# fahmyadan/SMARTS

Hardware: AMD Instinct MI355X
Metric: aggregate env-steps/s (all agents) (higher is better)
Workload: dtype f64; 1 GPU; scenarios/loop, 4096 batched envs x 32 Laner agents, waypoints(4x20, lookahead 32)+neighbours(10, r=50 m) obs, OGM 64x64 @ 50/64 m/px, dt=0.1, auto-reset (BASELINE.json configs[3]); total_envs=4096, envs_per_gpu=4096, vehicles_per_env=32, launch_form=large_one_lane

## Files before the change

### smarts_amd/csrc/smx_kernels.hip

```cpp
#include <hip/hip_runtime.h>

#include <algorithm>
#include <cmath>
#include <cstdio>
#include <cstdlib>
#include <cstring>
#include <new>
#include <string>
#include <vector>

#include "smx_guard.h"
#include "smx_history.h"
#include "smx_host.h"
#include "smx_plan.h"
#include "smx_scan.h"
#include "smx_vehicle.h"

#define SMX_COLLISION_LEEWAY 0.05
#define SMX_POSE_SCAN_RADIUS 10.0
#define SMX_WPT_PRELOAD 8
#define SMX_SLOW_BLOCKS 512

struct KernelArgs {
  smx_config cfg;
  MapDev map;
  smx_state st;
  smx_spawns sp;
  smx_outputs out;
  const int8_t* actions;
  const float* actions_f32;
  const double* traj;
  const int32_t* traj_n;
  int traj_max;
  const uint8_t* env_mask;
  const double* lidar_rays;
  const smx_via* vias;
  const int32_t* via_slot_off;
  int first_only;
  int keep_reward_done;
  int reset_all;
  double heading_gain_pos, lateral_gain_pos;
  int wp_pool_limit;
  char* wp_spill;
  int walk_new;
  double nb_d2_max;
  int debug_skip;
  int wp_blocks, obs_blocks, lidar_blocks;
  double dagm_reach;
  uint8_t* rgb;
  KnotLists knots;
  const KnotRow* knot_table;
  unsigned long long* knot_served;
  MissionsDev missions;
  const int32_t* alive_list;
  const int32_t* alive_count;
  int alive_segmented;
  int32_t* status;
  double* seeds_carry;
  double* facts_carry;
  int32_t* slow_list;
  int32_t* slow_count;
  uint8_t* seed_pending;
  uint8_t* guard;
  GuardBox guard_box;
  HistoryDev history;
  HistoryDimsDev dims;
};
enum {
  SMX_DEVICE_BAD_LANE_ACTION = 1,
  SMX_DEVICE_BAD_TRAJECTORY = 2,
  SMX_DEVICE_BAD_TARGET_POSE = 4
};

#define SF(field) a.st.f64[(size_t)(field) * total + gid]

#define SMX_SEG_STRIDE 32
__device__ __forceinline__ size_t seg_position(const size_t seg, const size_t off) {
  return ((off >> 6) << 9) | (seg << 6) | (off & 63);
}

__device__ __forceinline__ size_t launch_vehicle(const KernelArgs& a, size_t i, size_t total) {
  if (a.alive_list == nullptr) return i < total ? i : total;
  const int32_t entry = a.alive_list[i < total ? i : total - 1];
  if (a.alive_segmented) {
// ... 1060 lines not shown
              const double d = first_waypoint_distance(rx[q], ry[q], rdx[q], rdy[q], kn_n[q], px, py);
              if (d < my_d) {
                my_d = d;
                my_idx = __popc(started);
              }
              started |= 1 << q;
            }
          }
          const int n_paths = __popc(started);
          if (!slow && n_paths > 0) {
            const int want = wanted_path(my_idx, la.lane_change, n_paths);
#pragma unroll
            for (int q = 0; q < SMX_WP_LANES; ++q)
              if ((started >> q) & 1)
                if (__popc(started & ((1 << q) - 1)) == want) qw = q;
            int n32w = 0, nk16 = 0, last = -1, stw = 0;
            smx_lp_rec r0 = smx_lp_rec{};
#pragma unroll
            for (int q = 0; q < SMX_WP_LANES; ++q)
              if (q == qw) {
                stw = st[q];
                n32w = kn_n[q];
                nk16 = kn_nk16[q];
                last = kn_end16[q];
                r0.x = rx[q];
                r0.y = ry[q];
                r0.dirx = rdx[q];
                r0.diry = rdy[q];
                r0.heading = rh[q];
              }
            r0.lane = 0;
            const int n16 = n32w < SMX_CTRL_WPS ? n32w : SMX_CTRL_WPS;
            double* col = path_lds + threadIdx.x;
            const int32_t* const knot1 = table ? a.knot_table[stw].idx : a.knots.idx + paths + gid * SMX_WP_LANES + qw;
            ctrl_waypoints_from_knots<true>(a, knot1, table ? (size_t)1 : paths, r0, nk16, last, n16, px, py,
                                            [&](int i, const WaypointOut& w) {
                                              col[(size_t)i * SMX_BLOCK] = w.heading;
                                              if (i < CTRL_XY) {
                                                col[(size_t)(SMX_CTRL_WPS + i) * SMX_BLOCK] = w.x;
                                                col[(size_t)(SMX_CTRL_WPS + CTRL_XY + i) * SMX_BLOCK] = w.y;
                                              }
                                            });
            path.n = n16;
#pragma unroll
            for (int k = 0; k < SMX_CTRL_WPS; ++k) {
              const bool held = k < n16;
              path.h[k] = held ? col[(size_t)k * SMX_BLOCK] : 0.0;
              path.x[k] = (held && k < CTRL_XY) ? col[(size_t)(SMX_CTRL_WPS + (k < CTRL_XY ? k : 0)) * SMX_BLOCK] : 0.0;
              path.y[k] = (held && k < CTRL_XY) ? col[(size_t)(SMX_CTRL_WPS + CTRL_XY + (k < CTRL_XY ? k : 0)) * SMX_BLOCK] : 0.0;
            }
          }
        }
      }
      if (!slow) {
        ControlOut co = idle_command(cs);
        if (has_action) {
          if (path.n > 0 && !SMX_SKIP(a, 1 << 28)) {
            co = lane_following_from_path(s, cs, c.dt, la.target_speed, la.lane_change, la.hg, la.lg, path);
          } else {
            co = last_command(cs);
          }
        }
        SF(SMX_S_PREV_X) = s.x;
        SF(SMX_S_PREV_Y) = s.y;
        if (!SMX_SKIP(a, 1 << 27)) vehicle_step(s, co, c.dt);
        if (!GUARD || guard_before_store(a, gid, flags, s)) store_vehicle_state(a, gid, total, s, cs, flags);
      }
    }
  }
  const unsigned long long mask = __ballot(slow);
  if (mask != 0ull) {
    const int lane = threadIdx.x & 63;
    int base = 0;
    if (lane == __ffsll((long long)mask) - 1) base = atomicAdd(a.slow_count, __popcll(mask));
    base = __shfl(base, __ffsll((long long)mask) - 1);
// ... 756 lines not shown
  const size_t path = gid * SMX_WP_LANES + p0;
  const int flags = a.st.flags[gid];
  int n = 0, nk = 0, cnt = 0;
  double D = 0.0;
  if (honour_pending && a.seed_pending != nullptr && a.seed_pending[gid]) return;
  if ((flags & SMX_F_ALIVE) && !(flags & SMX_F_SOCIAL) && (!a.first_only || whatever_the_pass || (flags & SMX_F_FIRST))) {
    const PathSeeds seed = load_seeds(a, gid, total);
    if (seed.road >= 0 && seed.n_lanes <= SMX_WP_LANES && p0 < seed.n_lanes) {
      const double px = SF(SMX_S_X), py = SF(SMX_S_Y);
      const int start = seed_start(m, seed, p0, px, py);
      if (start >= 0) {
        a.knots.idx[path] = start;
        const KnotListHead w = walk_knot_list(m, seed.f, start, c.wp_lookahead, SMX_CTRL_WPS, px, py,
                                              [&](int k, int idx, double) { a.knots.idx[(size_t)k * paths + path] = idx; });
        n = w.n;
        nk = w.nk;
        D = w.D;
        cnt = w.cnt;
        a.knots.nk16[path] = (uint8_t)w.nk16;
        a.knots.end16[path] = w.end16;
        a.knots.key[path] = start;
        a.knots.key[paths + path] = seed.f.n > 0 ? seed.f.road[0] : -1;
        a.knots.key[2 * paths + path] = seed.f.n > 1 ? seed.f.road[1] : -1;
      }
    }
  }
  a.knots.n[path] = (int16_t)n;
  a.knots.nk[path] = (int16_t)nk;
  a.knots.cnt[path] = (uint8_t)cnt;
  a.knots.D[path] = D;
  if (n == 0) a.knots.key[path] = -1;
}

__global__ void __launch_bounds__(SMX_BLOCK) k_knot_table(const MapDev m, const int lookahead, KnotRow* rows, int32_t* stats) {
  const int lp = (int)(blockIdx.x * SMX_BLOCK + threadIdx.x);
  if (lp >= m.n_lanepoints) return;
  KnotRow row;
  build_knot_row(m, lp, lookahead, SMX_CTRL_WPS, row);
  rows[lp] = row;
  if (row.flags & SMX_KROW_TABLED) atomicAdd(stats, 1);
  if (row.flags & SMX_KROW_SINGLE_ROAD) atomicAdd(stats + 1, 1);
}

__global__ void __launch_bounds__(SMX_BLOCK) k_wp_walk(const KernelArgs a) {
  SMX_TSTAMP(span0);
  const size_t total = (size_t)a.cfg.num_envs * a.cfg.num_vehicles;
  const size_t lane_no = (size_t)blockIdx.x * SMX_BLOCK + threadIdx.x;
  wp_walk_for(a, launch_vehicle(a, lane_no / SMX_WP_LANES, total), (int)(lane_no % SMX_WP_LANES), true);
  SMX_TSTAMP(span1);
  SMX_TSPAN(3, span0, span1);
}

__global__ void __launch_bounds__(SMX_BLOCK) k_wp_walk_listed(const KernelArgs a) {
  const int count = *a.slow_count;
  constexpr int VPB = SMX_BLOCK / SMX_WP_LANES;
  for (int i = (int)blockIdx.x * VPB + (int)threadIdx.x / SMX_WP_LANES; i < count; i += (int)gridDim.x * VPB)
    wp_walk_for(a, (size_t)a.slow_list[i], (int)threadIdx.x % SMX_WP_LANES, false);
}

struct __align__(16) WpStageCell {
  float heading, width, speed;
  short lane;
  signed char lane_index;
  signed char pad;
};

__device__ __forceinline__ void waypoints_tables_role(const KernelArgs& a, const int block) {
  extern __shared__ __align__(16) unsigned char stage_raw[];
  __shared__ WpRowBook book;
  const smx_config& c = a.cfg;
  const MapDev& m = a.map;
  const smx_outputs& o = a.out;
// ... 156 lines not shown
      } else {
        n_paths_total = wp_emit_branches<SMX_BLOCK>(a, seed.f, gid, p0, px, py, knots, cnt > 0 ? a.knots.idx[path] : -1, cnt, -1, g);
        fw = team_first_waypoint(tm.started, g, n_paths_total > 0);
      }
      wp_close_rows(a, gid, p0, n_paths_total);
    } else {
      if (tm.staged && !tm.listed) {
        BranchState bs;
        bs.reset();
        wp_emit_path<SMX_BLOCK>(a, seed.f, bs, a.knots.idx[path], gid, px, py, knots, tm.my_row ? tm.prov : 0, tm.my_row, true, &g, false);
      }
      fw = team_first_waypoint(tm.started, g, tm.n_paths > 0);
    }
  }
  SMX_TSTAMP(tw5);
  SMX_TACC(5, tw4, tw5);
  if (live && p0 == 0) trip_meter_update<SMX_BLOCK>(a, gid, total, flags, px, py, knots, fw);
  SMX_TSTAMP(tw6);
  SMX_TACC(3, tw0, tw6);
}

#define SMX_WPE_KNOTS 10
#ifndef SMX_WPE_POOL
#define SMX_WPE_POOL 352
#endif
struct __align__(8) WpKnot {
  double x, y, h, cum;
};
struct WpKnotLanes {
  short lane, strict;
};
#define SMX_WPE_SPILL_GROUP_BYTES ((size_t)SMX_BLOCK * (SMX_WPE_KNOTS + 1) * (sizeof(WpKnot) + sizeof(WpKnotLanes)))

__device__ __forceinline__ void waypoints_emit_role(const KernelArgs& a, const int block) {
  __shared__ WpKnot pool[SMX_WPE_POOL];
  __shared__ WpKnotLanes pool_lanes[SMX_WPE_POOL];
  __shared__ WpRowBook book;
  __shared__ double hdr_step[SMX_BLOCK], hdr_D[SMX_BLOCK];
  __shared__ unsigned short hdr_off[SMX_BLOCK];
  __shared__ unsigned char hdr_nrec[SMX_BLOCK], hdr_n[SMX_BLOCK];
  __shared__ float hdr_w0[SMX_BLOCK], hdr_s0[SMX_BLOCK];
  __shared__ signed char hdr_li0[SMX_BLOCK];
  __shared__ unsigned char hdr_one_lane[SMX_BLOCK];
  __shared__ double first_wp[SMX_WPT_VEHICLES][3];
  __shared__ unsigned char rows_live[SMX_WPT_VEHICLES * SMX_WPT_MAX_PATHS], rows_zero[SMX_WPT_VEHICLES * SMX_WPT_MAX_PATHS];
  __shared__ unsigned char rows_spill[SMX_WPT_VEHICLES * SMX_WPT_MAX_PATHS];
  __shared__ unsigned char hdr_spill[SMX_BLOCK];
  static_assert(SMX_WPT_VEHICLES * SMX_WPT_MAX_PATHS <= 256, "row numbers are bytes");
  static_assert(sizeof(WpKnot) == 32 && sizeof(WpKnotLanes) == 4, "WpKnot layout");
  const smx_config& c = a.cfg;
  const MapDev& m = a.map;
  const smx_outputs& o = a.out;
  const size_t total = (size_t)c.num_envs * c.num_vehicles;
  const int P = c.wp_paths, W = c.wp_len;
  const int p0 = threadIdx.x % SMX_WP_LANES, v = threadIdx.x / SMX_WP_LANES;
  const size_t gid = launch_vehicle(a, (size_t)block * SMX_WPT_VEHICLES + v, total);
  const size_t path = gid * SMX_WP_LANES + p0, paths = total * SMX_WP_LANES;
  const int col = threadIdx.x;
  constexpr int KP = SMX_WPE_KNOTS;
  SMX_TSTAMP(te0);
  const bool in_range = gid < total;
  const size_t g = in_range ? gid : 0, pth = g * SMX_WP_LANES + p0;
  int flags = a.st.flags[g];
  const int pend = a.seed_pending != nullptr ? (int)a.seed_pending[g] : 0;
  double px = a.st.f64[(size_t)SMX_S_X * total + g], py = a.st.f64[(size_t)SMX_S_Y * total + g];
  PathSeeds seed = load_seeds(a, g, total);
  const bool table = a.knot_table != nullptr;
  int n_first, nk, cnt, kid0;
  double D = 0.0;
  int kid[KP];
  constexpr int KD = 6;
  double kd[KD];
  bool untabled = false;
  if (table) {
    kid0 = (seed.road >= 0 && seed.n_lanes <= SMX_WP_LANES && p0 < seed.n_lanes) ? seed_start(m, seed, p0, px, py) : -1;
    if ((unsigned)kid0 >= (unsigned)m.n_lanepoints) kid0 = -1;
    const KnotRow* row = a.knot_table + (kid0 >= 0 ? kid0 : 0);
    const bool serves = knot_row_serves(row->flags, row->f0, row->f1, row->road, seed.f);
    untabled = kid0 >= 0 && !serves;
    n_first = (kid0 >= 0 && serves) ? (int)row->n : 0;
    nk = (kid0 >= 0 && serves) ? (int)row->nk : 0;
    cnt = (kid0 >= 0 && serves) ? 1 : 0;
#pragma unroll
    for (int k = 0; k < KP; ++k) kid[k] = row->idx[k];
#pragma unroll
    for (int k = 0; k < KD; ++k) kd[k] = row->d[k];
    if (kid0 < 0) kid0 = 0;
  } else {
    n_first = a.knots.n[pth];
    nk = a.knots.nk[pth];
    cnt = a.knots.cnt[pth];
    D = a.knots.D[pth];
    kid0 = a.knots.idx[pth];
#pragma unroll
    for (int k = 0; k < KP; ++k) kid[k] = a.knots.idx[(size_t)(k + 1) * paths + pth];
#pragma unroll
    for (int k = 0; k < KD; ++k) kd[k] = 0.0;
  }
  const double trip_dist = a.st.f64[(size_t)SMX_S_DIST * total + g], trip_x = a.st.f64[(size_t)SMX_S_TRIP_X * total + g],
               trip_y = a.st.f64[(size_t)SMX_S_TRIP_Y * total + g], trip_h = a.st.f64[(size_t)SMX_S_TRIP_H * total + g];
  const int trip_has = a.st.facts_i32[(size_t)SMX_FI_TRIP_HAS_WP * total + g];
  const bool live = in_range && (flags & SMX_F_ALIVE) && !(flags & SMX_F_SOCIAL) && (!a.first_only || (flags & SMX_F_FIRST)) && !pend;
  if (!live) {
    seed.road = -1;
    seed.n_lanes = 0;
    seed.f.none();
    n_first = nk = cnt = 0;
    D = 0.0;
    untabled = false;
  }
  const bool seeded = live && seed.road >= 0;
  const WpTeam tm = wp_team_number(seeded, seed.n_lanes, p0, n_first, nk, cnt, P);
  SMX_TSTAMP(te1);
  SMX_TACC(32, te0, te1);
  bool tabled_path = false;
  int nrec = 0;
  double kx[KP], ky[KP], kh[KP], cum[KP];
  int kl[KP], kstrict[KP];
  double k0x = 0.0, k0y = 0.0, k0h = 0.0;
  int lane0 = 0;
#pragma unroll
  for (int k = 0; k < KP; ++k) {
    kx[k] = ky[k] = kh[k] = cum[k] = 0.0;
    kl[k] = kstrict[k] = 0;
  }
  const bool walk = tm.my_row && tm.listed && !SMX_SKIP(a, 1 << 22);
  if (walk) {
    const smx_lp_rec r0 = load_lp(m, kid0, 46);
    lane0 = r0.lane;
    const int nkp = nk < KP ? nk : KP;
    {
#pragma unroll
      for (int k = 0; k < KP; ++k) {
        const bool have = k < nkp;
        const smx_lp_rec* r = m.lp_rec + (have ? kid[k] : 0);
        kx[k] = have ? r->x : 0.0;
        ky[k] = have ? r->y : 0.0;
        kh[k] = have ? r->heading : 0.0;
        kl[k] = have ? r->lane : 0;
      }
    }
    const int n = n_first;
    if (n == 1) {
      k0x = r0.x;
      k0y = r0.y;
      k0h = r0.heading;
      nrec = 1;
      tabled_path = true;
    } else {
      const double proj = (px - r0.x) * r0.dirx + (py - r0.y) * r0.diry;
      k0x = r0.x + proj * r0.dirx;
      k0y = r0.y + proj * r0.diry;
      k0h = r0.heading;
      if (table) {
        const double ex = kx[0] - k0x, ey = ky[0] - k0y;
        D = sqrt(ex * ex + ey * ey);
#pragma unroll
        for (int k = 2; k <= KD + 1; ++k)
          if (k <= nk) D += kd[k - 2];
        const double* const rest = a.knot_table[kid0].d;
#pragma unroll 4
        for (int k = KD + 2; k <= nk; ++k) D += rest[k - 2];
      }
      const int n_emit = n < W ? n : W;
      const double step = D / (double)(n - 1);
      const double t_last = (n_emit - 1 == n - 1) ? D : (double)(n_emit - 1) * step;
      double jx = k0x, jy = k0y, jcum = 0.0;
      int jlane = lane0, strict_lane = lane0;
      Unwrap uw;
      uw.start(k0h);
      int need = -1;
#pragma unroll
      for (int k = 0; k < KP; ++k) {
        if (k < nkp && need < 0) {
          const double ex = kx[k] - jx, ey = ky[k] - jy;
          const double qcum = jcum + sqrt(ex * ex + ey * ey);
          kh[k] = uw.push(kh[k]);
          cum[k] = qcum;
          if (qcum > jcum) strict_lane = jlane;
          kstrict[k] = strict_lane;
          if (t_last < qcum) need = k + 2;
          jx = kx[k];
          jy = ky[k];
          jcum = qcum;
          jlane = kl[k];
        }
      }
      if (need < 0 && nkp == nk) need = nk + 1;
      if (need > 0) {
        nrec = need;
        tabled_path = true;
      }
    }
  }
  SMX_TSTAMP(te2);
  SMX_TACC(33, te1, te2);
  int incl = tabled_path ? nrec : 0;
  {
    const int lane = threadIdx.x & 63;
#pragma unroll
    for (int d = 1; d < 64; d <<= 1) {
      const int t = __shfl_up(incl, d);
      if (lane >= d) incl += t;
    }
  }
  const int off = incl - (tabled_path ? nrec : 0);
  const bool spilled = tabled_path && off + nrec > a.wp_pool_limit && a.wp_spill != nullptr;
// ... 2238 lines not shown
          dagm_role(a, (int)(g0 + j));
          __syncthreads();
        }
        if (c.sensors & SMX_SENSOR_RGB) {
          rgb_role(a, (int)(g0 + j));
          __syncthreads();
        }
      }
    }
  }
  if (t.list) {
    const size_t s0 = (g0 >> 6) & 7;
    const size_t seg = (gid >> 6) & 7;
    const unsigned long long m0 = __ballot(alive && seg == s0), m1 = __ballot(alive && seg != s0);
    int b0 = 0, b1 = 0;
    if (lane == 0) {
      if (m0) b0 = atomicAdd(t.seg_count + SMX_SEG_STRIDE * s0, __popcll(m0));
      if (m1) b1 = atomicAdd(t.seg_count + SMX_SEG_STRIDE * (((g1 - 1) >> 6) & 7), __popcll(m1));
    }
    b0 = __shfl(b0, 0);
    b1 = __shfl(b1, 0);
    const unsigned long long below = (1ull << lane) - 1ull;
    if (alive) {
      const bool first_seg = seg == s0;
      const size_t off = (size_t)(first_seg ? b0 : b1) + __popcll((first_seg ? m0 : m1) & below);
      t.list[seg_position(seg, off)] = (int32_t)gid;
    }
  }
}
__global__ void __launch_bounds__(SMX_BLOCK) k_waypoints(const KernelArgs a) { waypoints_role(a, (int)blockIdx.x); }
__global__ void __launch_bounds__(SMX_BLOCK) k_waypoints_tables(const KernelArgs a) { waypoints_tables_role(a, (int)blockIdx.x); }
__global__ void __launch_bounds__(SMX_BLOCK) k_waypoints_emit(const KernelArgs a) {
  SMX_TSTAMP(span0);
  waypoints_emit_role(a, (int)blockIdx.x);
  SMX_TSTAMP(span1);
  SMX_TSPAN(4, span0, span1);
}
__global__ void __launch_bounds__(SMX_BLOCK) k_waypoints_listed(const KernelArgs a) {
  __shared__ int knot_scratch[SMX_MAX_KNOTS * SMX_BLOCK];
  const int count = *a.slow_count;
  constexpr int VPB = SMX_BLOCK / SMX_WP_LANES;
  for (int i = (int)blockIdx.x * VPB + (int)threadIdx.x / SMX_WP_LANES; i < count; i += (int)gridDim.x * VPB)
    waypoints_for<SMX_BLOCK>(a, (size_t)a.slow_list[i], knot_scratch + threadIdx.x);
}
__global__ void __launch_bounds__(SMX_BLOCK) k_waypoints_walk_listed(const KernelArgs a) {
  __shared__ int knot_scratch[SMX_MAX_KNOTS * SMX_BLOCK];
  const int count = *a.slow_count;
  constexpr int VPB = SMX_BLOCK / (2 * SMX_WP_LANES);
  const bool walker = ((threadIdx.x / SMX_WP_LANES) & 1) != 0;
  for (int i = (int)blockIdx.x * VPB + (int)threadIdx.x / (2 * SMX_WP_LANES); i < count; i += (int)gridDim.x * VPB) {
    const size_t gid = (size_t)a.slow_list[i];
    if (walker)
      wp_walk_for(a, gid, (int)threadIdx.x % SMX_WP_LANES, false);
    else
      waypoints_for<SMX_BLOCK>(a, gid, knot_scratch + threadIdx.x);
  }
}
__global__ void __launch_bounds__(SMX_BLOCK) k_observe(const KernelArgs a) {
  SMX_TSTAMP(span0);
  observe_role(a, (int)blockIdx.x);
  SMX_TSTAMP(span1);
  SMX_TSPAN(5, span0, span1);
}
template <bool SIZED>
__global__ void __launch_bounds__(SMX_BLOCK) k_lidar(const KernelArgs a) { lidar_role<SIZED ? 1 : 0>(a, (int)blockIdx.x); }
#define SMX_LIDAR_FIRST_BLOCKS 1024
template <bool SIZED>
// ... 50 lines not shown
  if (!sel) return;
  a.st.env_episode[env] = a.st.env_episode[env] + 1;
  a.st.env_done_count[env] = 0;
  a.st.env_ticks[env] = c.reset_elapsed_steps;
  a.st.env_reset_pending[env] = 0;
  if (!a.keep_reward_done) a.out.env_done[env] = 0;
}

static double radius_threshold(double radius) {
  if (!(radius >= 0.0)) return -1.0;
  if (std::isinf(radius)) return radius;
  double t = radius * radius;
  if (std::isinf(t)) return t;
  while (t > 0.0 && std::sqrt(t) > radius) t = std::nextafter(t, 0.0);
  for (;;) {
    const double up = std::nextafter(t, INFINITY);
    if (std::isinf(up) || !(std::sqrt(up) <= radius)) break;
    t = up;
  }
  return t;
}

struct smx_handle_s {
  smx_config cfg;
  int device;
  bool map_loaded;
  MapDev map;
  void* map_blob;
  size_t map_bytes;
  void* knots_blob;
  void* spill_blob;
  int wp_pool_limit = SMX_WPE_POOL;
  KnotRow* knot_table;
  int32_t* knot_stats;
  int knot_table_mode = 1;
  int32_t* alive_blob;
  uint8_t* pending_blob;
  int32_t* slow_blob;
  double* scan_carry;
  int alive_parity;
  KnotLists knots;
  void* ctrl_blob;
  CtrlHandoff ctrl;
  int32_t* status_dev;
  hipStream_t side[3];
  hipEvent_t ev_fork, ev_fork_grid, ev_join[3];
  bool side_ready;
  const double* lidar_rays;
  smx_via* vias_dev;
  int32_t* via_off_dev;
  int32_t n_vias;
  void* missions_blob;
  std::vector<int32_t> host_lane_road, host_lane_out_off, host_lane_out_idx;
  void* goals_blob;
  std::vector<int32_t> host_route_last;
  MissionsDev missions;
  double heading_gain_pos = 0.04, lateral_gain_pos = 3.4;
  double nb_d2_max;
  int slow_blocks = SMX_SLOW_BLOCKS;
  bool list_ready;
  int seg_parity;
  smx_state list_state;
  int group_parity;
  bool map_junctions;
  double dagm_reach;
  uint8_t* guard_out;
// ... 224 lines not shown
    const size_t n = (size_t)h->cfg.num_envs * h->cfg.num_vehicles;
    SMX_HIP(hipMalloc((void**)&h->pending_blob, n));
    SMX_HIP(hipMemset(h->pending_blob, 0, n));
  }
  if (!h->scan_carry) {
    const size_t n = 6 * (size_t)h->cfg.num_envs * h->cfg.num_vehicles;
    SMX_HIP(hipMalloc((void**)&h->scan_carry, n * sizeof(double)));
    SMX_HIP(hipMemset(h->scan_carry, 0xff, n * sizeof(double)));
  }
  if ((h->cfg.sensors & SMX_SENSOR_WAYPOINTS) && !h->knots_blob) {
    const size_t paths = (size_t)h->cfg.num_envs * h->cfg.num_vehicles * SMX_WP_LANES;
    const size_t off_D = (size_t)(SMX_WPK_CAP + 1) * paths * sizeof(int32_t);
    const size_t off_n = off_D + paths * sizeof(double), off_nk = off_n + paths * sizeof(int16_t);
    const size_t off_end = off_nk + paths * sizeof(int16_t), off_key = off_end + paths * sizeof(int32_t);
    const size_t off_cnt = off_key + 3 * paths * sizeof(int32_t), off_nk16 = off_cnt + paths;
    const size_t bytes = off_nk16 + paths;
    SMX_HIP(hipMalloc(&h->knots_blob, bytes));
    SMX_HIP(hipMemset(h->knots_blob, 0, bytes));
    SMX_HIP(hipMemset((char*)h->knots_blob + off_key, 0xff, 3 * paths * sizeof(int32_t)));
    char* kb = (char*)h->knots_blob;
    h->knots.idx = (int32_t*)kb;
    h->knots.D = (double*)(kb + off_D);
    h->knots.n = (int16_t*)(kb + off_n);
    h->knots.nk = (int16_t*)(kb + off_nk);
    h->knots.end16 = (int32_t*)(kb + off_end);
    h->knots.key = (int32_t*)(kb + off_key);
    h->knots.cnt = (uint8_t*)(kb + off_cnt);
    h->knots.nk16 = (uint8_t*)(kb + off_nk16);
  }
  if (h->knot_table) {
    (void)hipFree(h->knot_table);
    h->knot_table = nullptr;
  }
  if (h->cfg.sensors & SMX_SENSOR_WAYPOINTS) {
    if (!h->knot_stats) SMX_HIP(hipMalloc((void**)&h->knot_stats, 4 * sizeof(int32_t)));
    SMX_HIP(hipMemset(h->knot_stats, 0, 4 * sizeof(int32_t)));
    SMX_HIP(hipMalloc((void**)&h->knot_table, (size_t)t->n_lanepoints * sizeof(KnotRow)));
    hipLaunchKernelGGL(k_knot_table, dim3(smx_blocks((size_t)t->n_lanepoints)), dim3(SMX_BLOCK), 0, 0, h->map, (int)h->cfg.wp_lookahead,
                       h->knot_table, h->knot_stats);
    SMX_HIP(hipGetLastError());
    SMX_HIP(hipDeviceSynchronize());
  }
  if ((h->cfg.sensors & SMX_SENSOR_WAYPOINTS) && !h->spill_blob) {
    const size_t tv = (size_t)h->cfg.num_envs * h->cfg.num_vehicles;
    const size_t groups = (tv + SMX_WPT_VEHICLES - 1) / SMX_WPT_VEHICLES;
    SMX_HIP(hipMalloc(&h->spill_blob, groups * SMX_WPE_SPILL_GROUP_BYTES));
  }
  if (!h->status_dev) {
    SMX_HIP(hipMalloc((void**)&h->status_dev, sizeof(int32_t)));
    SMX_HIP(hipMemset(h->status_dev, 0, sizeof(int32_t)));
  }
  if (!h->ctrl_blob) {
    const size_t tv = (size_t)h->cfg.num_envs * h->cfg.num_vehicles;
    const size_t path_bytes = (size_t)SMX_CTRL_WPS * 3 * tv * sizeof(double);
    SMX_HIP(hipMalloc(&h->ctrl_blob, path_bytes + tv * sizeof(int32_t)));
    SMX_HIP(hipMemset(h->ctrl_blob, 0, path_bytes + tv * sizeof(int32_t)));
    h->ctrl.path = (double*)h->ctrl_blob;
    h->ctrl.n = (int32_t*)((char*)h->ctrl_blob + path_bytes);
  }
  if (!h->side_ready) {
    int prio_least = 0, prio_greatest = 0;
    SMX_HIP(hipDeviceGetStreamPriorityRange(&prio_least, &prio_greatest));
    for (int i = 0; i < 3; ++i) {
      SMX_HIP(hipStreamCreateWithPriority(&h->side[i], hipStreamNonBlocking, ((SMX_SIDE_PRIO >> i) & 1) ? 0 : prio_least));
      SMX_HIP(hipEventCreateWithFlags(&h->ev_join[i], hipEventDisableTiming));
    }
    SMX_HIP(hipEventCreateWithFlags(&h->ev_fork, hipEventDisableTiming));
    SMX_HIP(hipEventCreateWithFlags(&h->ev_fork_grid, hipEventDisableTiming));
    h->side_ready = true;
  }
  h->guard_box = guard_box_of(*t, h->guard_margin);
  h->map_loaded = true;
// ... 483 lines not shown
  } else if (p.facts_start == FactsStart::AFTER_SEEDS) {
    if (p.chain() != SlowChain::SIDE) (void)hipEventRecord(h->ev_fork, stream);
    (void)hipStreamWaitEvent(s_obs, h->ev_fork, 0);
  }
  const KernelArgs kf = with_slow(k, p.facts_slow);
  switch (p.facts) {
    case Facts::SCAN: break;
    case Facts::ONE_LANE:
      launch(k_scan_fast<0>, p.facts_blocks, 0, s_obs, kf);
      launch(k_scan_listed<0>, p.slow_blocks, 0, s_obs, kf);
      break;
    case Facts::WIDE: launch(k_scan_half<0, false, SMX_TEAM>, p.facts_blocks, 0, s_obs, kf); break;
    case Facts::FOUR: launch(k_scan_half<0>, p.facts_blocks, 0, s_obs, kf); break;
  }
  if (ph) (void)hipEventRecord(ph[SMX_PHASE_SCAN + 1], stream);
  if (!p.fork) launch_grids(h, p, k, stream);
  if (ph) (void)hipEventRecord(ph[SMX_PHASE_OGM + 1], stream);
  KernelArgs kw = k;
  kw.seed_pending = p.seed_pending();
  const unsigned walk_blocks = smx_blocks(total * SMX_WP_LANES);
  switch (p.rows) {
    case Rows::SENSORS: launch(k_sensors, p.sensor_blocks, p.sensor_lds, stream, k); break;
    case Rows::UNSTAGED: launch(k_waypoints, p.wp_blocks, 0, stream, k); break;
    case Rows::TABLES:
      launch(k_wp_walk, walk_blocks, 0, stream, kw);
      launch(k_waypoints_tables, p.wp_blocks, std::max((size_t)h->cfg.wp_len * SMX_BLOCK * 16, (size_t)SMX_MAX_KNOTS * SMX_BLOCK * sizeof(int)),
             stream, k);
      break;
    case Rows::EMIT:
    case Rows::EMIT_CHAIN_SIDE:
    case Rows::EMIT_CHAIN_AFTER:
      if (!p.knot_table) launch(k_wp_walk, walk_blocks, 0, stream, kw);
      kw = with_slow(kw, p.rows_slow);
      launch(k_waypoints_emit, p.wp_blocks, 0, stream, kw);
      launch(k_waypoints_listed, p.slow_blocks, 0, stream, kw);
      if (p.rows == Rows::EMIT_CHAIN_AFTER) launch_slow_chain(p, ks, stream);
      break;
  }
  if (!p.small()) launch(k_observe, p.obs_blocks, 0, s_obs, k);
  if (p.lidar == Lidar::CALLER) launch(p.sized ? k_lidar<true> : k_lidar<false>, p.lidar_blocks, 0, stream, k);
  if (p.fork) {
    for (int i = 0; i < (p.chain() == SlowChain::SIDE ? 3 : 2); ++i) {
      (void)hipEventRecord(h->ev_join[i], h->side[i]);
      (void)hipStreamWaitEvent(stream, h->ev_join[i], 0);
    }
  }
  if (p.road_waypoints)
    launch(k_road_waypoints, smx_blocks(total * SMX_RW_LANE_CAP), 0, stream, k);
  if (p.lane_ttc)
    hipLaunchKernelGGL(k_lane_ttc, dim3(p.ttc_blocks), dim3(SMX_BLOCK), p.ttc_lds, stream, k, (const int32_t*)nullptr, (const int32_t*)nullptr);
  if (p.ego_centric)
    hipLaunchKernelGGL(k_ego_frame, dim3(p.ec_blocks), dim3(SMX_BLOCK), 0, stream, k, (const int32_t*)nullptr, (const int32_t*)nullptr);
  if (ph) (void)hipEventRecord(ph[SMX_PHASE_SENSORS + 1], stream);
}

static int tail_and_reset_pass(smx_handle h, const TickPlan& p, const KernelArgs& a, const uint8_t* mask, const smx_state* st,
                               hipStream_t stream, hipEvent_t* ph) {
  const size_t total = (size_t)h->cfg.num_envs * h->cfg.num_vehicles;
  const AliveLayout al = alive_layout(h->cfg);
  KernelArgs r = a;
  r.alive_list = nullptr;
  r.alive_count = nullptr;
  r.alive_segmented = 0;
  r.first_only = 1;
  r.keep_reward_done = p.is_step ? 1 : 0;
  r.reset_all = (!p.is_step && mask == nullptr) ? 1 : 0;
  r.env_mask = p.is_step ? nullptr : mask;
// ... 41 lines not shown

static KernelArgs kernel_args(smx_handle h, const TickPlan& p, const int8_t* actions, const float* actions_f32, const double* traj,
                              const int32_t* traj_n, int32_t traj_max, const uint8_t* mask, const smx_state* st, const smx_spawns* sp,
                              const smx_outputs* out) {
  const size_t total = (size_t)h->cfg.num_envs * h->cfg.num_vehicles;
  KernelArgs a;
  a.cfg = h->cfg;
  a.map = h->map;
  a.st = *st;
  a.sp = *sp;
  a.out = *out;
  a.actions = actions;
  a.actions_f32 = actions_f32;
  a.traj = traj;
  a.traj_n = traj_n;
  a.traj_max = traj_max;
  a.env_mask = mask;
  a.lidar_rays = h->lidar_rays;
  a.vias = h->n_vias > 0 ? h->vias_dev : nullptr;
  a.missions = h->missions;
  a.via_slot_off = h->via_off_dev;
  a.first_only = 0;
  a.keep_reward_done = 0;
  a.reset_all = 0;
  a.heading_gain_pos = h->heading_gain_pos;
  a.nb_d2_max = h->nb_d2_max;
  a.walk_new = 0;
  a.wp_spill = (char*)h->spill_blob;
  a.wp_pool_limit = h->wp_pool_limit;
  a.lateral_gain_pos = h->lateral_gain_pos;
  a.debug_skip = h->debug_skip;
  a.knots = h->knots;
  a.knot_table = p.knot_table ? h->knot_table : nullptr;
  a.knot_served = (p.knot_table && h->knot_table_mode == 2) ? (unsigned long long*)(h->knot_stats + 2) : nullptr;
  a.status = h->status_dev;
  a.alive_list = nullptr;
  a.alive_count = nullptr;
  a.alive_segmented = 0;
  a.slow_list = nullptr;
  a.slow_count = nullptr;
  a.seed_pending = nullptr;
  a.seeds_carry = h->scan_carry;
  a.facts_carry = h->scan_carry ? h->scan_carry + 4 * total : nullptr;
  a.dagm_reach = h->dagm_reach;
  a.rgb = h->rgb_out;
  a.guard = h->guard_out;
  a.guard_box = h->guard_box;
  a.history = h->history;
  a.dims = h->dims;
  a.wp_blocks = (int)p.wp_blocks;
  a.obs_blocks = (int)p.obs_blocks;
  a.lidar_blocks = (int)p.lidar_blocks;
  return a;
}

enum class Entry { RESET, LANE, FLOATS, TRAJECTORY, TARGET_POSE, TRAJECTORY_WITH_TIME };
static int enqueue(smx_handle h, const Entry entry, const int8_t* actions, const float* actions_f32, const double* traj,
                   const int32_t* traj_n, int32_t traj_max, const uint8_t* mask, const smx_state* st,
                   const smx_spawns* sp, const smx_outputs* out, void* stream_) {
  if (!h) return SMX_ERR_INVALID;
  if (!h->map_loaded) return fail(h, SMX_ERR_STATE, "smx_load_map has not been called");
  int rc = check_buffers(h, st, sp, out);
  if (rc != SMX_OK) return rc;
  const bool is_step = entry != Entry::RESET;
  if (is_step) {
    const int sp_ = h->cfg.action_space;
// ... 141 lines not shown
      if (bits & SMX_DEVICE_BAD_TRAJECTORY)
        return fail(h, SMX_ERR_INVALID,
                    "an illegal TrajectoryWithTime action reached smx_step_trajectory_with_time since the last smx_sync (fewer "
                    "than two points or more than max_points, a value that is not finite, times not strictly increasing, no "
                    "point later than dt or the first one already later); the agents that sent one were not moved");
      if (bits & SMX_DEVICE_BAD_TARGET_POSE)
        return fail(h, SMX_ERR_INVALID,
                    "a TargetPose action whose pose is not finite reached smx_step_target_pose, or an Imitation action "
                    "with an infinite component or a pose or speed that is not finite reached smx_step_continuous, since the "
                    "last smx_sync; the agents that sent one were stepped as if they had sent no action");
    }
  }
  return SMX_OK;
}

extern "C" int smx_debug_slow_counts(smx_handle h, int32_t* out4) {
  if (!h || !out4) return SMX_ERR_INVALID;
  if (!h->slow_blob) return fail(h, SMX_ERR_STATE, "no slow lists (the map is not loaded)");
  SMX_HIP(hipDeviceSynchronize());
  const size_t total = (size_t)h->cfg.num_envs * h->cfg.num_vehicles;
  SMX_HIP(hipMemcpy(out4, SlowLists{h->slow_blob, total}.counters(h->alive_parity ^ 1), 4 * sizeof(int32_t), hipMemcpyDeviceToHost));
  return SMX_OK;
}

extern "C" int smx_debug_set_wp_pool(smx_handle h, int32_t records) {
  if (!h) return SMX_ERR_INVALID;
  if (records < 1 || records > SMX_WPE_POOL) return fail(h, SMX_ERR_INVALID, "smx_debug_set_wp_pool: 1 .. SMX_WPE_POOL records");
  h->wp_pool_limit = records;
  return SMX_OK;
}

extern "C" int smx_debug_set_knot_table(smx_handle h, int32_t mode) {
  if (!h) return SMX_ERR_INVALID;
  if (mode < 0 || mode > 2) return fail(h, SMX_ERR_INVALID, "smx_debug_set_knot_table: 0 (walked lists), 1 (table), 2 (table, counting)");
  h->knot_table_mode = mode;
  return SMX_OK;
}

extern "C" int smx_debug_knot_table_stats(smx_handle h, int64_t* out4) {
  if (!h || !out4) return SMX_ERR_INVALID;
  if (!h->knot_table) return fail(h, SMX_ERR_STATE, "no knot table (no map loaded, or no waypoints sensor)");
  SMX_HIP(hipDeviceSynchronize());
  int32_t st[4];
  SMX_HIP(hipMemcpy(st, h->knot_stats, sizeof(st), hipMemcpyDeviceToHost));
  unsigned long long served;
  std::memcpy(&served, st + 2, sizeof(served));
  out4[0] = h->map.n_lanepoints;
  out4[1] = st[0];
  out4[2] = st[1];
  out4[3] = (int64_t)served;
  return SMX_OK;
}

extern "C" int smx_set_timing(smx_handle h, int level) {
  if (!h) return SMX_ERR_INVALID;
  h->timing = level == 1;
  h->phase_timing = level == 2;
  return SMX_OK;
}

extern "C" int smx_read_phase_ms(smx_handle h, float* ms, int32_t max_steps, int32_t* n) {
  if (!h || !ms || !n || max_steps < 0) return SMX_ERR_INVALID;
  int32_t count = 0;
  for (size_t i = 0; i < h->ph_used; ++i) {
    hipEvent_t* ph = &h->ph_pool[i * (SMX_PHASE_COUNT + 1)];
    SMX_HIP(hipEventSynchronize(ph[SMX_PHASE_COUNT]));
    if (count >= max_steps) continue;
    for (int p = 0; p < SMX_PHASE_COUNT; ++p) {
      float t = 0.f;
      SMX_HIP(hipEventElapsedTime(&t, ph[p], ph[p + 1]));
      ms[(size_t)count * SMX_PHASE_COUNT + p] = t;
    }
    ++count;
  }
  h->ph_used = 0;
  *n = count;
  return SMX_OK;
}

extern "C" int smx_read_step_ms(smx_handle h, float* ms, int32_t max, int32_t* n) {
  if (!h || !ms || !n || max < 0) return SMX_ERR_INVALID;
  int32_t count = 0;
  for (size_t i = 0; i < h->ev_used; ++i) {
    SMX_HIP(hipEventSynchronize(h->ev_pool[2 * i + 1]));
    float t = 0.f;
    SMX_HIP(hipEventElapsedTime(&t, h->ev_pool[2 * i], h->ev_pool[2 * i + 1]));
    if (count < max) ms[count++] = t;
  }
  h->ev_used = 0;
  *n = count;
  return SMX_OK;
}

extern "C" int smx_last_step_ms(smx_handle h, float* ms) {
  if (!h || !ms) return SMX_ERR_INVALID;
  if (h->ev_used == 0) return fail(h, SMX_ERR_STATE, "no timed step recorded (smx_set_timing(1) then smx_step)");
  const size_t i = h->ev_used - 1;
  SMX_HIP(hipEventSynchronize(h->ev_pool[2 * i + 1]));
  SMX_HIP(hipEventElapsedTime(ms, h->ev_pool[2 * i], h->ev_pool[2 * i + 1]));
  return SMX_OK;
}

extern "C" const char* smx_last_error(smx_handle h) { return h ? h->err.c_str() : g_create_err.c_str(); }

extern "C" void smx_destroy(smx_handle h) {
  if (!h) return;
  if (h->map_blob) (void)hipFree(h->map_blob);
  if (h->knots_blob) (void)hipFree(h->knots_blob);
  if (h->alive_blob) (void)hipFree(h->alive_blob);
  if (h->scan_carry) (void)hipFree(h->scan_carry);
  if (h->slow_blob) (void)hipFree(h->slow_blob);
  if (h->pending_blob) (void)hipFree(h->pending_blob);
  if (h->spill_blob) (void)hipFree(h->spill_blob);
  if (h->knot_table) (void)hipFree(h->knot_table);
  if (h->knot_stats) (void)hipFree(h->knot_stats);
  if (h->ctrl_blob) (void)hipFree(h->ctrl_blob);
  if (h->status_dev) (void)hipFree(h->status_dev);
  if (h->side_ready) {
    for (int i = 0; i < 3; ++i) {
      (void)hipStreamSynchronize(h->side[i]);
      (void)hipStreamDestroy(h->side[i]);
      (void)hipEventDestroy(h->ev_join[i]);
    }
    (void)hipEventDestroy(h->ev_fork);
    (void)hipEventDestroy(h->ev_fork_grid);
  }
  if (h->vias_dev) (void)hipFree(h->vias_dev);
  if (h->via_off_dev) (void)hipFree(h->via_off_dev);
  if (h->missions_blob) (void)hipFree(h->missions_blob);
  if (h->goals_blob) (void)hipFree(h->goals_blob);
  if (h->history_blob) (void)hipFree(h->history_blob);
  if (h->dims_blob) (void)hipFree(h->dims_blob);
  for (hipEvent_t e : h->ev_pool) (void)hipEventDestroy(e);
  for (hipEvent_t e : h->ph_pool) (void)hipEventDestroy(e);
  delete h;
}
```

### smarts_amd/csrc/smx_roadmap.h

```cpp
#pragma once
#include "smx_device.h"

#define SMX_INF 1.0e300

__device__ __forceinline__ smx_lp_rec load_lp(const MapDev& m, int i, int site = 1) {
  return m.lp_rec[SMX_BCHK(site, i, m.n_lanepoints)];
}

struct RoadFacts {
  int lane;
  double dist;
  bool on_road;
  int corner_mask;
};

__device__ inline RoadFacts road_facts_scan(const MapDev& m, double px, double py, double radius, int n_corners,
                                            const double* cx, const double* cy) {
  RoadFacts out;
  out.lane = -1;
  out.dist = SMX_INF;
  out.on_road = false;
  out.corner_mask = 0;
  const double road_radius = fmax(5.0, 2.0 * m.default_lane_width);
  int cx0 = (int)floor((px - radius - m.sg_x0) / m.sg_cell);
// ... 904 lines not shown

__device__ __forceinline__ RouteFilter knot_row_filter(const MapDev& m, int lp) {
  const int road = m.lane_road[m.lp_rec[lp].lane];
  RouteFilter f;
  f.none();
  if (m.road_is_junction[road]) f = junction_filter(m, road);
  return f;
}

__device__ inline void build_knot_row(const MapDev& m, int lp, int lookahead, int ctrl_wps, KnotRow& row) {
  const smx_lp_rec r0 = m.lp_rec[lp];
  const RouteFilter f = knot_row_filter(m, lp);
  const int road = m.lane_road[r0.lane];
  for (int k = 0; k < SMX_WPK_CAP; ++k) row.idx[k] = lp;
  for (int k = 0; k < SMX_WPK_CAP - 1; ++k) row.d[k] = 0.0;
  bool single = true;
  const KnotListHead hd = walk_knot_list(m, f, lp, lookahead, ctrl_wps, r0.x, r0.y, [&](int k, int idx, double term) {
    row.idx[k - 1] = idx;
    if (k >= 2) row.d[k - 2] = term;
    single = single && m.lane_road[m.lp_rec[idx].lane] == road;
  });
  const bool tabled = hd.cnt == 1 && hd.n > 0 && hd.nk <= SMX_WPK_CAP;
  row.n = (int16_t)hd.n;
  row.nk = (int16_t)hd.nk;
  row.nk16 = (uint8_t)hd.nk16;
  row.flags = (uint8_t)((tabled ? SMX_KROW_TABLED : 0) | (tabled && single ? SMX_KROW_SINGLE_ROAD : 0));
  row.pad = 0;
  row.end16 = hd.end16;
  row.f0 = f.n > 0 ? f.road[0] : -1;
  row.f1 = f.n > 1 ? f.road[1] : -1;
  row.road = road;
}

__device__ __forceinline__ bool knot_row_serves(int flags, int f0, int f1, int road, const RouteFilter& f) {
  if (!(flags & SMX_KROW_TABLED) || f.n == SMX_ROUTE_FIXED) return false;
  if (f0 == (f.n > 0 ? f.road[0] : -1) && f1 == (f.n > 1 ? f.road[1] : -1)) return true;
  return f0 < 0 && (flags & SMX_KROW_SINGLE_ROAD) && f.n > 0 && f.last() == road;
}
```

Measured before the change: 10.83 million env-steps/s.

## Precompute per-lanepoint knot records to avoid gathered lanepoint loads in waypoint emit

```diff
diff --git a/smarts_amd/csrc/smx_kernels.hip b/smarts_amd/csrc/smx_kernels.hip
--- a/smarts_amd/csrc/smx_kernels.hip
+++ b/smarts_amd/csrc/smx_kernels.hip
@@ -19,6 +19,9 @@
 #define SMX_COLLISION_LEEWAY 0.05
 #define SMX_POSE_SCAN_RADIUS 10.0
 #define SMX_WPT_PRELOAD 8
+#ifndef SMX_CTRL_RECORDS
+#define SMX_CTRL_RECORDS 0
+#endif
 #define SMX_SLOW_BLOCKS 512
 
 struct KernelArgs {
@@ -50,6 +53,7 @@
   uint8_t* rgb;
   KnotLists knots;
   const KnotRow* knot_table;
+  const KnotRecRow* knot_recs;
   unsigned long long* knot_served;
   MissionsDev missions;
   const int32_t* alive_list;
@@ -1176,15 +1180,21 @@
             r0.lane = 0;
             const int n16 = n32w < SMX_CTRL_WPS ? n32w : SMX_CTRL_WPS;
             double* col = path_lds + threadIdx.x;
-            const int32_t* const knot1 = table ? a.knot_table[stw].idx : a.knots.idx + paths + gid * SMX_WP_LANES + qw;
-            ctrl_waypoints_from_knots<true>(a, knot1, table ? (size_t)1 : paths, r0, nk16, last, n16, px, py,
-                                            [&](int i, const WaypointOut& w) {
-                                              col[(size_t)i * SMX_BLOCK] = w.heading;
-                                              if (i < CTRL_XY) {
-                                                col[(size_t)(SMX_CTRL_WPS + i) * SMX_BLOCK] = w.x;
-                                                col[(size_t)(SMX_CTRL_WPS + CTRL_XY + i) * SMX_BLOCK] = w.y;
-                                              }
-                                            });
+            auto put = [&](int i, const WaypointOut& w) {
+              col[(size_t)i * SMX_BLOCK] = w.heading;
+              if (i < CTRL_XY) {
+                col[(size_t)(SMX_CTRL_WPS + i) * SMX_BLOCK] = w.x;
+                col[(size_t)(SMX_CTRL_WPS + CTRL_XY + i) * SMX_BLOCK] = w.y;
+              }
+            };
+            if (SMX_CTRL_RECORDS && a.knot_recs != nullptr) {
+              const unsigned rw = (unsigned)stw < (unsigned)m.n_lanepoints ? (unsigned)stw : 0u;
+              ctrl_waypoints_from_records<SMX_WPT_PRELOAD>(m, a.knot_recs + rw, a.knot_table[rw].d, r0, nk16 < SMX_KREC_KNOTS ? nk16 : SMX_KREC_KNOTS,
+                                          last >= 0, n16, SMX_CTRL_WPS, px, py, put);
+            } else {
+              const int32_t* const knot1 = table ? a.knot_table[stw].idx : a.knots.idx + paths + gid * SMX_WP_LANES + qw;
+              ctrl_waypoints_from_knots<true>(a, knot1, table ? (size_t)1 : paths, r0, nk16, last, n16, px, py, put);
+            }
             path.n = n16;
 #pragma unroll
             for (int k = 0; k < SMX_CTRL_WPS; ++k) {
@@ -2007,12 +2017,14 @@
   if (n == 0) a.knots.key[path] = -1;
 }
 
-__global__ void __launch_bounds__(SMX_BLOCK) k_knot_table(const MapDev m, const int lookahead, KnotRow* rows, int32_t* stats) {
+__global__ void __launch_bounds__(SMX_BLOCK) k_knot_table(const MapDev m, const int lookahead, KnotRow* rows, KnotRecRow* recs,
+                                                           int32_t* stats) {
   const int lp = (int)(blockIdx.x * SMX_BLOCK + threadIdx.x);
   if (lp >= m.n_lanepoints) return;
   KnotRow row;
   build_knot_row(m, lp, lookahead, SMX_CTRL_WPS, row);
   rows[lp] = row;
+  build_knot_records(m, lp, row, recs[lp]);
   if (row.flags & SMX_KROW_TABLED) atomicAdd(stats, 1);
   if (row.flags & SMX_KROW_SINGLE_ROAD) atomicAdd(stats + 1, 1);
 }
@@ -2235,6 +2247,7 @@
 };
 #define SMX_WPE_SPILL_GROUP_BYTES ((size_t)SMX_BLOCK * (SMX_WPE_KNOTS + 1) * (sizeof(WpKnot) + sizeof(WpKnotLanes)))
 
+template <bool RECS>
 __device__ __forceinline__ void waypoints_emit_role(const KernelArgs& a, const int block) {
   __shared__ WpKnot pool[SMX_WPE_POOL];
   __shared__ WpKnotLanes pool_lanes[SMX_WPE_POOL];
@@ -2268,13 +2281,18 @@
   const int pend = a.seed_pending != nullptr ? (int)a.seed_pending[g] : 0;
   double px = a.st.f64[(size_t)SMX_S_X * total + g], py = a.st.f64[(size_t)SMX_S_Y * total + g];
   PathSeeds seed = load_seeds(a, g, total);
-  const bool table = a.knot_table != nullptr;
+  const bool table = RECS || a.knot_table != nullptr;
   int n_first, nk, cnt, kid0;
   double D = 0.0;
   int kid[KP];
   constexpr int KD = 6;
   double kd[KD];
   bool untabled = false;
+  constexpr bool recs = RECS;
+  static_assert(SMX_WPE_KNOTS <= SMX_KREC_KNOTS, "a record row holds the knots a path lane keeps");
+  double kx[KP], ky[KP], kh[KP];
+  int kl[KP];
+  smx_lp_rec r0 = smx_lp_rec{};
   if (table) {
     kid0 = (seed.road >= 0 && seed.n_lanes <= SMX_WP_LANES && p0 < seed.n_lanes) ? seed_start(m, seed, p0, px, py) : -1;
     if ((unsigned)kid0 >= (unsigned)m.n_lanepoints) kid0 = -1;
@@ -2285,10 +2303,33 @@
     nk = (kid0 >= 0 && serves) ? (int)row->nk : 0;
     cnt = (kid0 >= 0 && serves) ? 1 : 0;
 #pragma unroll
-    for (int k = 0; k < KP; ++k) kid[k] = row->idx[k];
-#pragma unroll
-    for (int k = 0; k < KD; ++k) kd[k] = row->d[k];
+    for (int k = 0; k < KP; ++k) kid[k] = 0;
+#pragma unroll
+    for (int k = 0; k < KD; ++k) kd[k] = 0.0;
+    if (!recs) {
+#pragma unroll
+      for (int k = 0; k < KP; ++k) kid[k] = row->idx[k];
+#pragma unroll
+      for (int k = 0; k < KD; ++k) kd[k] = row->d[k];
+    }
     if (kid0 < 0) kid0 = 0;
+    if (recs) {
+      const KnotRecRow* rr = a.knot_recs + kid0;
+      const smx_lp_rec* s0 = m.lp_rec + kid0;
+      r0.x = s0->x;
+      r0.y = s0->y;
+      r0.heading = s0->heading;
+      r0.dirx = s0->dirx;
+      r0.diry = s0->diry;
+      r0.lane = s0->lane;
+#pragma unroll
+      for (int k = 0; k < KP; ++k) {
+        kx[k] = rr->k[k].x;
+        ky[k] = rr->k[k].y;
+        kh[k] = rr->k[k].h;
+        kl[k] = rr->k[k].lane;
+      }
+    }
   } else {
     n_first = a.knots.n[pth];
     nk = a.knots.nk[pth];
@@ -2318,21 +2359,25 @@
   SMX_TACC(32, te0, te1);
   bool tabled_path = false;
   int nrec = 0;
-  double kx[KP], ky[KP], kh[KP], cum[KP];
-  int kl[KP], kstrict[KP];
+  double cum[KP];
+  int kstrict[KP];
   double k0x = 0.0, k0y = 0.0, k0h = 0.0;
   int lane0 = 0;
 #pragma unroll
   for (int k = 0; k < KP; ++k) {
-    kx[k] = ky[k] = kh[k] = cum[k] = 0.0;
-    kl[k] = kstrict[k] = 0;
+    if (!recs) {
+      kx[k] = ky[k] = kh[k] = 0.0;
+      kl[k] = 0;
+    }
+    cum[k] = 0.0;
+    kstrict[k] = 0;
   }
   const bool walk = tm.my_row && tm.listed && !SMX_SKIP(a, 1 << 22);
   if (walk) {
-    const smx_lp_rec r0 = load_lp(m, kid0, 46);
+    if (!recs) r0 = load_lp(m, kid0, 46);
     lane0 = r0.lane;
     const int nkp = nk < KP ? nk : KP;
-    {
+    if (!recs) {
 #pragma unroll
       for (int k = 0; k < KP; ++k) {
         const bool have = k < nkp;
@@ -2355,7 +2400,23 @@
       k0x = r0.x + proj * r0.dirx;
       k0y = r0.y + proj * r0.diry;
       k0h = r0.heading;
-      if (table) {
+      if (recs) {
+        const double ex = kx[0] - k0x, ey = ky[0] - k0y;
+        double c = sqrt(ex * ex + ey * ey);
+        cum[0] = c;
+        const double* const rest = a.knot_table[kid0].d;
+        double term[KP];
+#pragma unroll
+        for (int k = 1; k < KP; ++k) term[k] = rest[k - 1];
+#pragma unroll
+        for (int k = 1; k < KP; ++k) {
+          if (k < nk) c += term[k];
+          cum[k] = c;
+        }
+#pragma unroll 4
+        for (int k = KP; k < nk; ++k) c += rest[k - 1];
+        D = c;
+      } else if (table) {
         const double ex = kx[0] - k0x, ey = ky[0] - k0y;
         D = sqrt(ex * ex + ey * ey);
 #pragma unroll
@@ -2375,7 +2436,16 @@
       int need = -1;
 #pragma unroll
       for (int k = 0; k < KP; ++k) {
-        if (k < nkp && need < 0) {
+        if (recs) {
+          if (k < nkp && need < 0) {
+            const double qcum = cum[k];
+            if (qcum > jcum) strict_lane = jlane;
+            kstrict[k] = strict_lane;
+            if (t_last < qcum) need = k + 2;
+            jcum = qcum;
+            jlane = kl[k];
+          }
+        } else if (k < nkp && need < 0) {
           const double ex = kx[k] - jx, ey = ky[k] - jy;
           const double qcum = jcum + sqrt(ex * ex + ey * ey);
           kh[k] = uw.push(kh[k]);
@@ -4680,7 +4750,13 @@
 __global__ void __launch_bounds__(SMX_BLOCK) k_waypoints_tables(const KernelArgs a) { waypoints_tables_role(a, (int)blockIdx.x); }
 __global__ void __launch_bounds__(SMX_BLOCK) k_waypoints_emit(const KernelArgs a) {
   SMX_TSTAMP(span0);
-  waypoints_emit_role(a, (int)blockIdx.x);
+  waypoints_emit_role<true>(a, (int)blockIdx.x);
+  SMX_TSTAMP(span1);
+  SMX_TSPAN(4, span0, span1);
+}
+__global__ void __launch_bounds__(SMX_BLOCK) k_waypoints_emit_gather(const KernelArgs a) {
+  SMX_TSTAMP(span0);
+  waypoints_emit_role<false>(a, (int)blockIdx.x);
   SMX_TSTAMP(span1);
   SMX_TSPAN(4, span0, span1);
 }
@@ -4797,6 +4873,7 @@
   void* spill_blob;
   int wp_pool_limit = SMX_WPE_POOL;
   KnotRow* knot_table;
+  KnotRecRow* knot_recs;
   int32_t* knot_stats;
   int knot_table_mode = 1;
   int32_t* alive_blob;
@@ -5087,12 +5164,17 @@
     (void)hipFree(h->knot_table);
     h->knot_table = nullptr;
   }
+  if (h->knot_recs) {
+    (void)hipFree(h->knot_recs);
+    h->knot_recs = nullptr;
+  }
   if (h->cfg.sensors & SMX_SENSOR_WAYPOINTS) {
     if (!h->knot_stats) SMX_HIP(hipMalloc((void**)&h->knot_stats, 4 * sizeof(int32_t)));
     SMX_HIP(hipMemset(h->knot_stats, 0, 4 * sizeof(int32_t)));
     SMX_HIP(hipMalloc((void**)&h->knot_table, (size_t)t->n_lanepoints * sizeof(KnotRow)));
+    SMX_HIP(hipMalloc((void**)&h->knot_recs, (size_t)t->n_lanepoints * sizeof(KnotRecRow)));
     hipLaunchKernelGGL(k_knot_table, dim3(smx_blocks((size_t)t->n_lanepoints)), dim3(SMX_BLOCK), 0, 0, h->map, (int)h->cfg.wp_lookahead,
-                       h->knot_table, h->knot_stats);
+                       h->knot_table, h->knot_recs, h->knot_stats);
     SMX_HIP(hipGetLastError());
     SMX_HIP(hipDeviceSynchronize());
   }
@@ -5642,7 +5724,7 @@
     case Rows::EMIT_CHAIN_AFTER:
       if (!p.knot_table) launch(k_wp_walk, walk_blocks, 0, stream, kw);
       kw = with_slow(kw, p.rows_slow);
-      launch(k_waypoints_emit, p.wp_blocks, 0, stream, kw);
+      launch(kw.knot_recs != nullptr ? k_waypoints_emit : k_waypoints_emit_gather, p.wp_blocks, 0, stream, kw);
       launch(k_waypoints_listed, p.slow_blocks, 0, stream, kw);
       if (p.rows == Rows::EMIT_CHAIN_AFTER) launch_slow_chain(p, ks, stream);
       break;
@@ -5750,6 +5832,7 @@
   a.debug_skip = h->debug_skip;
   a.knots = h->knots;
   a.knot_table = p.knot_table ? h->knot_table : nullptr;
+  a.knot_recs = (p.knot_table && h->knot_table_mode != 3) ? h->knot_recs : nullptr;
   a.knot_served = (p.knot_table && h->knot_table_mode == 2) ? (unsigned long long*)(h->knot_stats + 2) : nullptr;
   a.status = h->status_dev;
   a.alive_list = nullptr;
@@ -5957,7 +6040,8 @@
 
 extern "C" int smx_debug_set_knot_table(smx_handle h, int32_t mode) {
   if (!h) return SMX_ERR_INVALID;
-  if (mode < 0 || mode > 2) return fail(h, SMX_ERR_INVALID, "smx_debug_set_knot_table: 0 (walked lists), 1 (table), 2 (table, counting)");
+  if (mode < 0 || mode > 3)
+    return fail(h, SMX_ERR_INVALID, "smx_debug_set_knot_table: 0 (walked lists), 1 (table), 2 (table, counting), 3 (table, no records)");
   h->knot_table_mode = mode;
   return SMX_OK;
 }
@@ -5977,6 +6061,14 @@
   return SMX_OK;
 }
 
+extern "C" int smx_debug_knot_table_bytes(smx_handle h, int64_t* out2) {
+  if (!h || !out2) return SMX_ERR_INVALID;
+  if (!h->knot_table || !h->knot_recs) return fail(h, SMX_ERR_STATE, "no knot table (no map loaded, or no waypoints sensor)");
+  out2[0] = (int64_t)h->map.n_lanepoints * (int64_t)sizeof(KnotRow);
+  out2[1] = (int64_t)h->map.n_lanepoints * (int64_t)sizeof(KnotRecRow);
+  return SMX_OK;
+}
+
 extern "C" int smx_set_timing(smx_handle h, int level) {
   if (!h) return SMX_ERR_INVALID;
   h->timing = level == 1;
@@ -6038,6 +6130,7 @@
   if (h->pending_blob) (void)hipFree(h->pending_blob);
   if (h->spill_blob) (void)hipFree(h->spill_blob);
   if (h->knot_table) (void)hipFree(h->knot_table);
+  if (h->knot_recs) (void)hipFree(h->knot_recs);
   if (h->knot_stats) (void)hipFree(h->knot_stats);
   if (h->ctrl_blob) (void)hipFree(h->ctrl_blob);
   if (h->status_dev) (void)hipFree(h->status_dev);
diff --git a/smarts_amd/csrc/smx_roadmap.h b/smarts_amd/csrc/smx_roadmap.h
--- a/smarts_amd/csrc/smx_roadmap.h
+++ b/smarts_amd/csrc/smx_roadmap.h
@@ -960,6 +960,200 @@
   row.road = road;
 }
 
+#define SMX_KREC_KNOTS 16
+struct KnotRec {
+  double x, y, h;
+  int32_t lane;
+  int32_t pad;
+};
+struct alignas(64) KnotRecRow {
+  KnotRec k[SMX_KREC_KNOTS];
+  KnotRec end;
+  double end_d;
+  double pad[3];
+};
+static_assert(sizeof(KnotRec) == 32 && sizeof(KnotRecRow) == 576, "KnotRecRow is nine 64-byte lines");
+
+__device__ inline void build_knot_records(const MapDev& m, int lp, const KnotRow& row, KnotRecRow& out) {
+  const smx_lp_rec r0 = m.lp_rec[lp];
+  const int nk = row.nk < SMX_KREC_KNOTS ? row.nk : SMX_KREC_KNOTS;
+  Unwrap uw;
+  uw.start(r0.heading);
+  for (int k = 0; k < SMX_KREC_KNOTS; ++k) {
+    KnotRec q;
+    q.x = q.y = q.h = 0.0;
+    q.lane = q.pad = 0;
+    if (k < nk) {
+      const smx_lp_rec r = m.lp_rec[row.idx[k]];
+      q.x = r.x;
+      q.y = r.y;
+      q.h = uw.push(r.heading);
+      q.lane = r.lane;
+    }
+    out.k[k] = q;
+  }
+  KnotRec e;
+  e.x = e.y = e.h = 0.0;
+  e.lane = e.pad = 0;
+  double end_d = 0.0;
+  const int nk16 = row.nk16;
+  if (row.end16 >= 0 && nk16 >= 1 && nk16 <= SMX_KREC_KNOTS && nk16 - 1 <= nk) {
+    const smx_lp_rec r = m.lp_rec[row.end16];
+    Unwrap u16;
+    u16.start(r0.heading);
+    for (int k = 0; k < nk16 - 1; ++k) (void)u16.push(m.lp_rec[row.idx[k]].heading);
+    e.x = r.x;
+    e.y = r.y;
+    e.h = u16.push(r.heading);
+    e.lane = r.lane;
+    if (nk16 >= 2) {
+      const smx_lp_rec b = m.lp_rec[row.idx[nk16 - 2]];
+      const double ex = r.x - b.x, ey = r.y - b.y;
+      end_d = sqrt(ex * ex + ey * ey);
+    }
+  }
+  out.end = e;
+  out.end_d = end_d;
+  out.pad[0] = out.pad[1] = out.pad[2] = 0.0;
+}
+
+template <int KP, class More, class Emit>
+__device__ __forceinline__ void interpolate_knot_records(const MapDev& m, const smx_lp_rec& r0, double w0, double s0, int nk, int n,
+                                                         double D, double px, double py, int max_emit, const double (&kx)[KP],
+                                                         const double (&ky)[KP], const double (&kh)[KP], const double (&kt)[KP],
+                                                         const int (&kl)[KP], const double (&kw)[KP], const double (&ks)[KP],
+                                                         More&& more, Emit&& emit) {
+  const int lane0 = r0.lane;
+  if (n == 1) {
+    if (max_emit > 0) {
+      WaypointOut o;
+      o.x = r0.x;
+      o.y = r0.y;
+      o.heading = r0.heading;
+      o.width = w0;
+      o.speed = s0;
+      o.lane = lane0;
+      emit(0, o);
+    }
+    return;
+  }
+  const int n_emit = min(n, max_emit);
+  if (n_emit <= 0) return;
+  const double proj = (px - r0.x) * r0.dirx + (py - r0.y) * r0.diry;
+  const double k0x = r0.x + proj * r0.dirx, k0y = r0.y + proj * r0.diry;
+  const double step = D / (double)(n - 1);
+  int i = 0;
+  double t = 0.0;
+  double jx = k0x, jy = k0y, jh = r0.heading, jcum = 0.0;
+  int jlane = lane0;
+  int strict_lane = lane0;
+  double wj = w0, sj = s0;
+  auto knot = [&](double qx, double qy, double qh, double term, int qlane, double wq, double sq) {
+    const double qcum = jcum + term;
+    if (i < n_emit && t < qcum) {
+      const double den = qcum - jcum;
+      const double sx = (qx - jx) / den, sy = (qy - jy) / den, sh = (qh - jh) / den;
+      double sw = 0.0, ss = 0.0;
+      if (qlane != jlane) {
+        sw = (wq - wj) / den;
+        ss = (sq - sj) / den;
+      }
+      do {
+        WaypointOut o;
+        const double dt_ = t - jcum;
+        o.x = sx * dt_ + jx;
+        o.y = sy * dt_ + jy;
+        o.heading = sh * dt_ + jh;
+        o.width = sw * dt_ + wj;
+        o.speed = ss * dt_ + sj;
+        const int dl = (t == jcum) ? strict_lane : jlane;
+        o.heading = wrap_heading(o.heading);
+        o.lane = dl;
+        emit(i, o);
+        ++i;
+        t = (i == n - 1) ? D : (double)i * step;
+      } while (i < n_emit && t < qcum);
+    }
+    if (qcum > jcum) strict_lane = jlane;
+    jx = qx;
+    jy = qy;
+    jh = qh;
+    jcum = qcum;
+    jlane = qlane;
+    wj = wq;
+    sj = sq;
+  };
+#pragma unroll
+  for (int k = 0; k < KP; ++k) {
+    if (k < nk && i < n_emit) {
+      const bool change = kl[k] != jlane;
+      knot(kx[k], ky[k], kh[k], kt[k], kl[k], change ? kw[k] : wj, change ? ks[k] : sj);
+    }
+  }
+  for (int k = KP; k < nk && i < n_emit; ++k) {
+    double qx, qy, qh, term;
+    int qlane;
+    more(k, qx, qy, qh, term, qlane);
+    double wq = wj, sq = sj;
+    if (qlane != jlane) {
+      wq = m.lane_width[SMX_BCHK(18, qlane, m.n_lanes)];
+      sq = m.lane_speed[qlane];
+    }
+    knot(qx, qy, qh, term, qlane, wq, sq);
+  }
+  while (i < n_emit) {
+    WaypointOut o;
+    o.x = jx;
+    o.y = jy;
+    o.heading = wrap_heading(jh);
+    o.width = wj;
+    o.speed = sj;
+    o.lane = (t > jcum) ? jlane : strict_lane;
+    emit(i, o);
+    ++i;
+    t = (i == n - 1) ? D : (double)i * step;
+  }
+}
+
+template <int KP, class Put>
+__device__ __forceinline__ void ctrl_waypoints_from_records(const MapDev& m, const KnotRecRow* rr, const double* rowd, const smx_lp_rec& r0,
+                                                            int nk16, bool ended, int n16, int ctrl_wps, double px, double py, Put&& put) {
+  static_assert(KP <= SMX_KREC_KNOTS && SMX_KREC_KNOTS - 1 <= SMX_WPK_CAP - 1, "a row's records and terms cover the controller's knots");
+  double kx[KP], ky[KP], kh[KP], kt[KP], kw[KP], ks_[KP];
+  int kl[KP];
+  auto rec_of = [&](int k) { return (k == nk16 - 1 && ended) ? &rr->end : &rr->k[k < SMX_KREC_KNOTS ? k : SMX_KREC_KNOTS - 1]; };
+  auto term_of = [&](int k) { return (k == nk16 - 1 && ended) ? &rr->end_d : &rowd[(k < SMX_KREC_KNOTS ? k : SMX_KREC_KNOTS - 1) - 1]; };
+#pragma unroll
+  for (int k = 0; k < KP; ++k) {
+    const KnotRec* r = rec_of(k);
+    kx[k] = r->x;
+    ky[k] = r->y;
+    kh[k] = r->h;
+    kt[k] = k > 0 ? *term_of(k) : 0.0;
+    kl[k] = 0;
+    kw[k] = ks_[k] = 0.0;
+  }
+  const double proj = (px - r0.x) * r0.dirx + (py - r0.y) * r0.diry;
+  const double ex = kx[0] - (r0.x + proj * r0.dirx), ey = ky[0] - (r0.y + proj * r0.diry);
+  kt[0] = sqrt(ex * ex + ey * ey);
+  double D = 0.0;
+#pragma unroll
+  for (int k = 0; k < KP; ++k)
+    if (k < nk16) D += kt[k];
+  for (int k = KP; k < nk16; ++k) D += *term_of(k);
+  interpolate_knot_records<KP>(
+      m, r0, 0.0, 0.0, nk16, n16, D, px, py, ctrl_wps, kx, ky, kh, kt, kl, kw, ks_,
+      [&](int k, double& qx, double& qy, double& qh, double& term, int& qlane) {
+        const KnotRec* r = rec_of(k);
+        qx = r->x;
+        qy = r->y;
+        qh = r->h;
+        term = *term_of(k);
+        qlane = 0;
+      },
+      put);
+}
+
 __device__ __forceinline__ bool knot_row_serves(int flags, int f0, int f1, int road, const RouteFilter& f) {
   if (!(flags & SMX_KROW_TABLED) || f.n == SMX_ROUTE_FIXED) return false;
   if (f0 == (f.n > 0 ? f.road[0] : -1) && f1 == (f.n > 1 ? f.road[1] : -1)) return true;
```

After: 10.79 million env-steps/s. Within noise of the previous version (-0.3%).
